# JacobMackay/beifong

Measured on AMD Instinct MI355X. Metric: Mrays/s (closest + any-hit BVH queries), Bus.obj-class radar scene, higher is better.
Workload: dtype f32

## Files before the change

### beifong_amd/csrc/bf_api.cpp

```cpp
#include <hip/hip_runtime.h>

#include <algorithm>
#include <atomic>
#include <cmath>
#include <cstdarg>
#include <cstdio>
#include <cstring>
#include <limits>
#include <memory>
#include <new>
#include <string>
#include <vector>

#include <dlfcn.h>
#if defined(__has_include) && __has_include(<rccl/rccl.h>)
#include <rccl/rccl.h>
#else
extern "C" {
typedef struct ncclComm *ncclComm_t;
typedef enum { ncclSuccess = 0 } ncclResult_t;
typedef enum { ncclFloat = 7 } ncclDataType_t;
typedef enum { ncclSum = 0 } ncclRedOp_t;
ncclResult_t ncclCommInitAll(ncclComm_t *comm, int ndev, const int *devlist);
ncclResult_t ncclCommDestroy(ncclComm_t comm);
// ... 13 lines not shown
#include "bf_wavefront.h"

extern "C" hipError_t bfk_launch_render(const bfd::DScene *sc, const bfd::DLaunch *lp, float *g_hist, bf_path_record *records,
                                        unsigned long long *counters, int stats, unsigned grid, size_t lds_bytes,
                                        hipStream_t stream);
extern "C" float bfk_host_cos(float x);
extern "C" hipError_t bfk_launch_translate(const float4 *tris0, float4 *tris, uint32_t n_tri_rows, const float4 *nodes0,
                                           float4 *nodes, float4 *qnodes, uint32_t n_nodes, const float4 *wnodes0, float4 *wnodes,
                                           uint32_t n_wchildren, const float *d, hipStream_t stream);
extern "C" hipError_t bfk_launch_rigid(const float4 *tris0, float4 *tris, const float4 *nrm0, float4 *nrm, uint32_t n_tris,
                                       const float *xf, const float4 *nodes0, float4 *nodes, float4 *qnodes, uint32_t n_nodes, const uint32_t *lvl4,
                                       const uint32_t *lvl4_off, uint32_t n_lvl4, float4 *ubox4, const float4 *wnodes0, float4 *wnodes, const uint32_t *lvl16,
                                       const uint32_t *lvl16_off, uint32_t n_lvl16, float4 *ubox16, float abs_pad, uint32_t n_versions,
                                       uint64_t vstride, uint32_t xf_stride, hipStream_t stream);
extern "C" hipError_t bfk_launch_elementary(int op, uint64_t n, const float *x, float *y);
extern "C" hipError_t bfk_launch_trace(const bfd::DScene *sc, uint64_t n, const float *rays, int any_hit, float *out_t,
                                       uint32_t *out_prim, uint32_t *out_shape, float *out_uv, uint8_t *out_hit,
                                       float *out_si, hipStream_t stream);
extern "C" hipError_t bfk_launch_query(int op, const bfd::DScene *sc, uint64_t n, const uint32_t *materials, uint32_t emitter,
                                       const float *in, float *out, hipStream_t stream);
extern "C" hipError_t bfk_launch_microfacet(int op, uint32_t type, float alpha_u, float alpha_v, uint32_t sample_visible, uint64_t n,
                                            const float *in, float *out, hipStream_t stream);

extern "C" hipError_t bfk_wf_shade(const bfd::DScene *sc, const bfd::DLaunch *lp, const bfd::WF *wf, uint32_t it, int first,
                                   float *g_hist, bf_path_record *records, unsigned grid, size_t lds_bytes,
                                   hipStream_t stream, int waves);
extern "C" hipError_t bfk_wf_trace(const bfd::DScene *sc, const bfd::WF *wf, uint32_t it, int stats, unsigned grid,
                                   hipStream_t stream, int waves);
extern "C" hipError_t bfk_launch_tail(const bfd::DScene *sc, const bfd::DLaunch *lp, const bfd::WF *wf, uint32_t it,
                                      uint32_t n_slots, float *g_hist, bf_path_record *records, int stats, size_t lds_bytes,
                                      hipStream_t stream, int tail_waves, unsigned spread, unsigned block_cap);
extern "C" hipError_t bfk_roll_set(bfd::DRoll *ring, float4 *offsets, uint32_t idx, const bfd::DRoll *d, const float *offset3, hipStream_t stream);
extern "C" hipError_t bfk_launch_render_fast(const bfd::DScene *sc, const bfd::DLaunch *lp, float *g_hist, bf_path_record *records,
                                             unsigned long long *counters, int stats, unsigned grid, size_t lds_bytes,
                                             hipStream_t stream);
extern "C" hipError_t bfk_wf_shade_fast(const bfd::DScene *sc, const bfd::DLaunch *lp, const bfd::WF *wf, uint32_t it, int first,
                                        float *g_hist, bf_path_record *records, unsigned grid, size_t lds_bytes,
                                        hipStream_t stream, int waves);
extern "C" hipError_t bfk_wf_trace_fast(const bfd::DScene *sc, const bfd::WF *wf, uint32_t it, int stats, unsigned grid,
                                        hipStream_t stream, int waves);
extern "C" hipError_t bfk_launch_tail_fast(const bfd::DScene *sc, const bfd::DLaunch *lp, const bfd::WF *wf, uint32_t it,
                                           uint32_t n_slots, float *g_hist, bf_path_record *records, int stats, size_t lds_bytes,
                                           hipStream_t stream, int tail_waves, unsigned spread, unsigned block_cap);

namespace {
struct Kernels {
    decltype(&bfk_launch_render) render;
    decltype(&bfk_wf_shade) shade;
    decltype(&bfk_wf_trace) trace;
    decltype(&bfk_launch_tail) tail;
};
const Kernels kExact = {bfk_launch_render, bfk_wf_shade, bfk_wf_trace, bfk_launch_tail};
const Kernels kFast = {bfk_launch_render_fast, bfk_wf_shade_fast, bfk_wf_trace_fast, bfk_launch_tail_fast};
const Kernels &kernels_for(uint32_t flags) { return (flags & BF_FLAG_FAST) ? kFast : kExact; }
}

namespace {

thread_local std::string g_err;
// ... 186 lines not shown
        uint32_t window = 1;
        uint32_t iters = 0;
        uint32_t flush_iters = 0;
        uint32_t flush_live = 0;
        bool multi = false;
        uint32_t fb_call_iters = 0;
        bool fb_is_flush = false;
    };
    mutable Roll roll;
    struct TabLayout {
        size_t o_rects = 0, o_shapes = 0, o_emit = 0, o_mat = 0, o_sensor = 0, stride = 0;
    };
    mutable TabLayout tab;
    mutable char *tab_pool = nullptr;
    mutable uint32_t tab_next = 0;
    mutable bool tables_in_pool = false;
    const bfd::DRect *home_rects = nullptr;
    const bfd::DShape *home_shapes = nullptr;
    const bfd::DEmitter *home_emitters = nullptr;
    const bfd::DMaterial *home_materials = nullptr;
    const bfd::DSensor *home_sensor = nullptr;
    mutable bfd::DRoll *roll_ring = nullptr;
    mutable float4 *roll_offsets = nullptr;
    struct WfPlan {
        bool valid = false;
        uint64_t n_paths = 0;
        uint32_t mode = 0, max_depth = 0, n_slots = 0, tail_max = 0;
        uint32_t iters = 0, tail_live = 0;
    };
    mutable WfPlan wf_plan;
    static constexpr int kStageSlots = 8;
    struct Stage {
        void *host = nullptr, *dev = nullptr;
        size_t cap = 0;
        hipEvent_t ev = nullptr;
        bool busy = false;
    };
    mutable Stage stage[kStageSlots];
    mutable int stage_next = 0;
    mutable uint32_t *wf_feedback = nullptr;
    mutable hipEvent_t wf_fb_event = nullptr;
    mutable bool wf_fb_pending = false;
    mutable uint32_t wf_fb_iters = 0;
};

namespace {
// ... 1138 lines not shown
    {
        hipError_t e = hipMalloc((void **) &sc->counters, sizeof(unsigned long long) * bfd::CTR_COUNT);
        if (e == hipSuccess) e = hipMemset(sc->counters, 0, sizeof(unsigned long long) * bfd::CTR_COUNT);
        if (e != hipSuccess) return fail_out(fail(BF_ERR_DEVICE, "bf_scene_clone: counters: %s", hipGetErrorString(e)));
    }
    sc->home_rects = sc->d.rects;
    sc->home_shapes = sc->d.shapes;
    sc->home_emitters = sc->d.emitters;
    sc->home_materials = sc->d.materials;
    sc->home_sensor = sc->d.sensor;
    *out = sc;
    return BF_OK;
}


static bf_status wf_ensure(const bf_scene *scene, uint32_t capacity) {
    bfd::WF &wf = scene->wf;
    if (wf.capacity >= capacity) return BF_OK;
    for (void *p : scene->wf_owned) (void) hipFree(p);
    scene->wf_owned.clear();
    std::memset(&wf, 0, sizeof(wf));
    scene->roll_ring = nullptr;
    scene->roll_offsets = nullptr;
    auto alloc = [&](void **p, size_t bytes) -> hipError_t {
        hipError_t e = hipMalloc(p, bytes);
        if (e == hipSuccess) scene->wf_owned.push_back(*p);
        return e;
    };
    size_t n = capacity, nb = capacity / 64;
#if BF_STATE_AOS
#if BF_STATE_AOS == 2
    HIP_TRY(alloc((void **) &wf.recA, n * 128));
    wf.recB = wf.recA + 4;
#else
    HIP_TRY(alloc((void **) &wf.recA, n * 64));
    HIP_TRY(alloc((void **) &wf.recB, n * 64));
#endif
    HIP_TRY(alloc((void **) &wf.recC, n * 64));
#else
    HIP_TRY(alloc((void **) &wf.ray0_, n * 16));
    HIP_TRY(alloc((void **) &wf.ray1_, n * 16));
    HIP_TRY(alloc((void **) &wf.sa_, n * 16));
    HIP_TRY(alloc((void **) &wf.sb_, n * 16));
    HIP_TRY(alloc((void **) &wf.sd_, n * 16));
    HIP_TRY(alloc((void **) &wf.se_, n * 16));
    HIP_TRY(alloc((void **) &wf.hit_, n * 16));
    HIP_TRY(alloc((void **) &wf.hit_prim_, n * 4));
    HIP_TRY(alloc((void **) &wf.sh0_, n * 16));
    HIP_TRY(alloc((void **) &wf.sh1_, n * 16));
    HIP_TRY(alloc((void **) &wf.sh2_, n * 4));
    HIP_TRY(alloc((void **) &wf.sh3_, n * 4));
    HIP_TRY(alloc((void **) &wf.render_, n * 4));
    HIP_TRY(alloc((void **) &wf.dop_, n * 4));
#endif
    HIP_TRY(alloc((void **) &scene->wf_masks, 8 * nb * sizeof(unsigned long long)));
    HIP_TRY(alloc((void **) &wf.n_live, (bfd::kWfMaxIter + 2) * sizeof(uint32_t)));
    HIP_TRY(alloc((void **) &scene->roll_ring, bfd::kRollRing * sizeof(bfd::DRoll)));
    HIP_TRY(alloc((void **) &scene->roll_offsets, bfd::kRollRing * sizeof(float4)));
    HIP_TRY(alloc((void **) &wf.surv_cursor, 64));
    wf.counters = scene->counters;
    wf.capacity = capacity;
    if (!scene->wf_host) HIP_TRY(hipHostMalloc((void **) &scene->wf_host, 64));
    if (!scene->wf_event) HIP_TRY(hipEventCreateWithFlags(&scene->wf_event, hipEventDisableTiming));
    if (!scene->wf_feedback) HIP_TRY(hipHostMalloc((void **) &scene->wf_feedback, (bfd::kWfMaxIter + 2) * sizeof(uint32_t)));
    if (!scene->wf_fb_event) HIP_TRY(hipEventCreateWithFlags(&scene->wf_fb_event, hipEventDisableTiming));
    scene->wf_plan.valid = false;
    scene->wf_fb_pending = false;
    return BF_OK;
}

static uint32_t wf_tail_threshold(const bf_scene *scene, uint32_t n_slots) {
    if (scene->tun.tail >= 0) return (uint32_t) scene->tun.tail;
    if (n_slots >= bfd::kTailSmallPool) return 1u << 17;
    return std::max<uint32_t>(1u << 17, std::min<uint32_t>(1u << 19, n_slots / 2));
}

namespace {
struct WfCtx {
    const bf_scene *scene;
    const Kernels *k;
    const bfd::DLaunch *lp;
// ... 86 lines not shown
    wf.rf_min = scene->tun.rf_min;
    wf.rf_th = scene->tun.rf_th;
    wf.rf_tm = scene->tun.rf_tm;
    c.lds_shade = ((sizeof(float) * lp.lds_floats + 15) & ~size_t(15)) + (scene->d.tab_cache ? bfd::kTabBytes : 0u);
    c.lds_tail = sizeof(int) * bfd::kStackDepth * bfd::kBlock + c.lds_shade;
    const unsigned batches_per_block = bfd::kBlock / 64;
    const unsigned max_blocks = (unsigned) ((nb + batches_per_block - 1) / batches_per_block);
    c.grid_shade = std::max(1u, std::min((unsigned) scene->n_cus * (unsigned) std::max(2, scene->tun.shade_waves), max_blocks));
    c.grid_trace = std::max(1u, std::min((unsigned) scene->n_cus * (unsigned) scene->tun.trace_waves, max_blocks));
    if (rolling && scene->tun.grid_share > 1u && wf.n_slots < scene->tun.grid_small) {
        const unsigned peers = (unsigned) std::max(1, scene->peers_rolling->load(std::memory_order_relaxed));
        const unsigned share = std::min(peers, (unsigned) scene->tun.grid_share);
        c.grid_shade = std::max(1u, c.grid_shade / share);
        c.grid_trace = std::max(1u, c.grid_trace / share);
    }
    c.tail_max = wf_tail_threshold(scene, rolling ? wf.n_main / 2 : wf.n_slots);
    wf.surv_claims_max = (wf.n_surv / 64u) / std::max(1u, c.grid_shade * batches_per_block);
    if (rolling && scene->tun.debug_surv_batches) {
        const char *e = getenv("BF_DEBUG_SURV_CLAIMS");
        wf.surv_claims_max = e ? (uint32_t) strtoul(e, nullptr, 10) : 1u << 20;
    }
    return BF_OK;
}
static bf_status wf_iteration(const WfCtx &c, uint32_t it, int first) {
    const bf_scene *scene = c.scene;
    const bfd::WF &wf = scene->wf;
    const int nxt = (it & 1) ^ 1;
    HIP_TRY(hipMemsetAsync(wf.m_alive[nxt], 0, c.mask_bytes, c.stream));
    if (first != 1) {
        HIP_TRY(wf_tic(c, 1));
        HIP_TRY(c.k->shade(&scene->d, c.lp, &wf, it, first == 2 ? 3 : 0, c.hist, c.rec, c.grid_shade, c.lds_shade, c.stream,
                           scene->tun.shade_waves));
        HIP_TRY(wf_toc(c));
    }
    if (first != 0) {
        HIP_TRY(wf_tic(c, 1));
        HIP_TRY(c.k->shade(&scene->d, c.lp, &wf, it, first, c.hist, c.rec, c.grid_shade, c.lds_shade, c.stream, scene->tun.shade_waves));
        HIP_TRY(wf_toc(c));
    }
    return BF_OK;
}
static bf_status wf_trace_launch(const WfCtx &c, uint32_t it) {
    HIP_TRY(wf_tic(c, 0));
    HIP_TRY(c.k->trace(&c.scene->d, &c.scene->wf, it, c.count_nodes ? 1 : 0, c.grid_trace, c.stream, c.scene->tun.trace_waves));
    HIP_TRY(wf_toc(c));
    return BF_OK;
}
static bf_status wf_tail_launch(const WfCtx &c, uint32_t it, uint32_t est_live, bool alone = false) {
    const bf_scene *scene = c.scene;
    uint32_t share = 1;
    if (!alone && scene->tun.tail_share > 1) {
        share = scene->tun.tail_share >= 4 ? 4u : 2u;
        est_live = (uint32_t) std::min<uint64_t>((uint64_t) est_live * share, 1u << 30);
    }
    if (alone) {
        const uint32_t resident = (uint32_t) scene->n_cus * 4u * 3u;
        while (share < 4u && (uint64_t) est_live * (share * 2u) / 64u <= resident) share *= 2u;
        est_live = (uint32_t) std::min<uint64_t>((uint64_t) est_live * share, 1u << 30);
    }
    scene->wf.tail_share = share;
// ... 1416 lines not shown
```

### beifong_amd/csrc/bf_device_core.h

```cpp
#pragma once
#include "bf_device.h"
#include "bf_device_math.h"

BF_NS_BEGIN

struct Hit {
    float t, u, v;
    uint32_t prim;
    int32_t slot;
};

BF_DEV bool tri_intersect(V3 p0, V3 p1, V3 p2, V3 o, V3 d, float mint, float maxt, float &t, float &u, float &v) {
    V3 e1 = p1 - p0, e2 = p2 - p0;
    V3 pvec = cross(d, e2);
    float inv_det = rcp(dot(e1, pvec));
    V3 tvec = o - p0;
    u = dot(tvec, pvec) * inv_det;
    bool active = u >= 0.f && u <= 1.f;
    V3 qvec = cross(tvec, e1);
    v = dot(d, qvec) * inv_det;
    active = active && v >= 0.f && u + v <= 1.f;
    t = dot(e2, qvec) * inv_det;
    return active && t >= mint && t <= maxt;
}
// ... 696 lines not shown
        }
        if (FULL) {
            geom->n = n;
            geom->dp_du = dp_du;
            geom->dp_dv = dp_dv;
        }
        if (tag & 1u) {
            si.sh.n = normalize(mk(na.x, na.y, na.z) * b0 + mk(nb.x, nb.y, nb.z) * b1 + mk(nc.x, nc.y, nc.z) * b2);
        } else {
            si.sh.n = n;
        }
    }
    float dd = dot(si.sh.n, dp_du);
    si.sh.s = normalize(mk(fnmadd(si.sh.n.x, dd, dp_du.x), fnmadd(si.sh.n.y, dd, dp_du.y), fnmadd(si.sh.n.z, dd, dp_du.z)));
    si.sh.t = cross(si.sh.n, si.sh.s);
    si.wi = to_local(si.sh, -d);
}

struct Microfacet {
    uint32_t type;
    float au, av;
    bool sample_visible;
};
BF_DEV void load_tables_lds(DScene &sc, uint32_t byte_off, uint32_t tid) {
    extern __shared__ __align__(16) unsigned char s_dyn[];
    sc.tab_on = 0u;
    if (!sc.tab_cache) return;
    float *dst = reinterpret_cast<float *>(s_dyn + byte_off);
    const float *gm = reinterpret_cast<const float *>(sc.materials), *gr = reinterpret_cast<const float *>(sc.rects);
    for (uint32_t i = tid; i < sc.n_materials * 12u; i += kBlock) dst[i] = gm[i];
    for (uint32_t i = tid; i < sc.n_rects * kRectDwords; i += kBlock) dst[kTabMaxMaterials * 12u + i] = gr[i];
    sc.lds_mat = byte_off;
    sc.lds_rect = byte_off + kTabMaxMaterials * 48u;
    sc.tab_on = 1u;
}
BF_DEV bf_material load_material(const DScene &sc, uint32_t index) {
    bf_f4 a, b, c;
    if (sc.tab_on) {
        extern __shared__ __align__(16) unsigned char s_dyn[];
        const lds_f4_ptr mp = (lds_f4_ptr) (s_dyn + sc.lds_mat) + 3u * index;
        a = mp[0], b = mp[1], c = mp[2];
    } else {
        const c_f4_ptr mp = (c_f4_ptr) (uintptr_t) (sc.materials + index);
        a = mp[0], b = mp[1], c = mp[2];
    }
    bf_material m;
    m.type = __float_as_uint(a.x);
    m.twosided = __float_as_uint(a.y);
    m.reflectance = a.z;
    m.alpha_u = a.w;
    m.alpha_v = b.x;
    m.distribution = __float_as_uint(b.y);
    m.sample_visible = __float_as_uint(b.z);
    m.eta = b.w;
    m.k = c.x;
    m.has_specular_reflectance = __float_as_uint(c.y);
    m.back_material = __float_as_uint(c.z);
// ... 338 lines not shown
```

### beifong_amd/csrc/bf_kernels.hip

```cpp
#include <algorithm>
#include <cstring>

#include "bf_path_logic.h"

BF_NS_BEGIN

#ifndef BF_TAIL_WAVES
#define BF_TAIL_WAVES 3
#endif
#ifdef BF_TAIL_PROF
__device__ unsigned long long g_tail_prof[8192 * 24];
#define BF_PROF_STAMP(var) const unsigned long long var = __builtin_amdgcn_s_memtime()
#else
#define BF_PROF_STAMP(var)
#endif
template <bool STATS, bool RESUME, bool SPILL, int TW = BF_TAIL_WAVES, int VX = 0>
__global__ __launch_bounds__(kBlock, RESUME ? TW : 3) void bf_render_kernel(DScene sc_arg, DLaunch lp, float *__restrict__ g_hist,
                                                           bf_path_record *__restrict__ records,
                                                           unsigned long long *__restrict__ counters, WF wf, uint32_t wf_it) {
    constexpr int kRX = 2 | VX;
    extern __shared__ __align__(16) unsigned char s_raw[];
    int *s_stack = reinterpret_cast<int *>(s_raw);
    float *s_hist = reinterpret_cast<float *>(s_raw + sizeof(int) * kStackDepth * kBlock);
    const int tid = threadIdx.x;
// ... 559 lines not shown
    if (MODE >= 1) row = (g * 2654435761u) & (n - 1u);
    if (MODE == 2) row *= 8u;
    const float4 v = table[row];
    if (v.x == 12345.678f) out[g & 1023u] = v;
}
BF_NS_END
extern "C" hipError_t bfk_gather_probe(int mode, const float4 *table, uint32_t n_rows, float4 *out, hipStream_t stream) {
    const uint32_t n = mode == 2 ? n_rows / 8u : n_rows;
    const dim3 grid((n + 255u) / 256u), block(256);
    if (mode == 0) hipLaunchKernelGGL(bfd::bf_gather_probe<0>, grid, block, 0, stream, table, n_rows, out);
    else if (mode == 1) hipLaunchKernelGGL(bfd::bf_gather_probe<1>, grid, block, 0, stream, table, n_rows, out);
    else hipLaunchKernelGGL(bfd::bf_gather_probe<2>, grid, block, 0, stream, table, n_rows, out);
    return hipGetLastError();
}

BF_NS_BEGIN
__global__ void bf_roll_set_kernel(DRoll *ring, float4 *offsets, uint32_t idx, DRoll d, float4 off) {
    if (threadIdx.x == 0 && blockIdx.x == 0) {
        ring[idx] = d;
        offsets[idx] = off;
    }
}
BF_NS_END
extern "C" hipError_t bfk_roll_set(bfd::DRoll *ring, float4 *offsets, uint32_t idx, const bfd::DRoll *d, const float *offset3, hipStream_t stream) {
    const float4 off = offset3 ? make_float4(offset3[0], offset3[1], offset3[2], 0.f) : make_float4(0.f, 0.f, 0.f, 0.f);
    hipLaunchKernelGGL(bfd::bf_roll_set_kernel, dim3(1), dim3(64), 0, stream, ring, offsets, idx, *d, off);
    return hipGetLastError();
}

BF_NS_BEGIN
BF_DEV void quantise_node4_dev(float4 lx, float4 ly, float4 lz, float4 hx, float4 hy, float4 hz, float4 refs, float4 *__restrict__ q) {
    const float cl[3][4] = {{lx.x, lx.y, lx.z, lx.w}, {ly.x, ly.y, ly.z, ly.w}, {lz.x, lz.y, lz.z, lz.w}};
    const float chh[3][4] = {{hx.x, hx.y, hx.z, hx.w}, {hy.x, hy.y, hy.z, hy.w}, {hz.x, hz.y, hz.z, hz.w}};
    const int child[4] = {__float_as_int(refs.x), __float_as_int(refs.y), __float_as_int(refs.z), __float_as_int(refs.w)};
    float nlo[3], scale[3];
    uint32_t exps = 0, qlo[3] = {0, 0, 0}, qhi[3] = {0, 0, 0};
    for (int a = 0; a < 3; ++a) {
        float lo = BF_INF, hi = -BF_INF;
        for (int k = 0; k < 4; ++k)
            if (child[k] != kNoNode) {
                lo = __builtin_fminf(lo, cl[a][k]);
                hi = __builtin_fmaxf(hi, chh[a][k]);
            }
        nlo[a] = lo;
        int e = 0;
        (void) __builtin_frexpf((hi - lo) * (1.f / 255.f), &e);
// ... 438 lines not shown
```

### beifong_amd/csrc/bf_wavefront.h

```cpp
#pragma once
#include <hip/hip_runtime.h>

#include "bf_ns.h"
#include <stdint.h>

BF_NS_BEGIN

constexpr uint32_t kWfMaxIter = 4096;
constexpr uint32_t kShadeChain = 8;
constexpr uint32_t kTraceRefill = 32;
constexpr uint32_t kTraceStragglers = 12;
constexpr uint32_t kTraceBlocksPerCU = 8;
constexpr uint32_t kTailSmallPool = 1u << 22;
constexpr uint32_t kTailRowJobs = 12;

#ifndef BF_STATE_AOS
#define BF_STATE_AOS 1
#endif
#define BF_HD __host__ __device__ __forceinline__

struct WF {
#if BF_STATE_AOS
    static constexpr size_t kAB = BF_STATE_AOS == 2 ? 8 : 4;
    float4 *recA, *recB, *recC;
    BF_HD float4 &ray0(uint32_t i) const { return recA[kAB * (size_t) i + 0]; }
    BF_HD float4 &ray1(uint32_t i) const { return recA[kAB * (size_t) i + 1]; }
    BF_HD float4 &hit(uint32_t i) const { return recA[kAB * (size_t) i + 2]; }
// ... 35 lines not shown
    uint32_t geom_stride;
    unsigned long long *m_alive[2];
    unsigned long long *m_trace[2];
    unsigned long long *m_shadow[2];
    unsigned long long *m_hit[2];
    uint32_t hit_split;
    uint32_t chain_min;
    uint32_t rf_min, rf_th, rf_tm;
    uint32_t *n_live;
    unsigned long long *counters;
    uint32_t trace_refill, trace_stragglers;
    uint32_t iq;
    uint32_t shade_chain;
    uint32_t row_jobs;
    uint32_t n_slots;
    uint32_t capacity;
    uint32_t n_main, n_surv;
    uint32_t *surv_cursor;
    uint32_t wake_b0, wake_nb;
    uint32_t tail_share;
    uint32_t surv_claims_max;
};

BF_NS_END
```

### beifong_amd/csrc/bf_wavefront.hip

```cpp
#include "bf_path_logic.h"

BF_NS_BEGIN

BF_DEV void publish_masks(unsigned long long *m_out, bool aligned, bool merge, uint32_t batch0, uint32_t slot, bool valid_lane, bool bit) {
    if (aligned) {
        unsigned long long w = __ballot(bit);
        if ((threadIdx.x & 63) == 0 && w) {
            if (merge)
                atomicOr(&m_out[batch0], w);
            else
                m_out[batch0] = w;
        }
    } else if (valid_lane && bit) {
        atomicOr(&m_out[slot >> 6], 1ull << (slot & 63u));
    }
}

constexpr uint32_t kPublishGroups = 4;
BF_DEV void publish_grouped(volatile unsigned char *tr, int lane, bool settle, uint32_t slot, uint32_t bits, unsigned long long *m_alive,
                            unsigned long long *m_trace, unsigned long long *m_shadow) {
    unsigned long long todo = __ballot(settle && bits != 0u);
    for (uint32_t n = 0; todo != 0ull && n < kPublishGroups; ++n) {
        const int j = __ffsll(todo) - 1;
        const uint32_t b = (uint32_t) __shfl((int) (slot >> 6), j);
// ... 79 lines not shown
            sv.free = 0ull;
        } else {
            const uint32_t p = nth_set_bit(sv.free, take - 1u);
            sv.free &= ~((2ull << p) - 1ull);
        }
        served += take;
    }
    if (evict && rank >= served) evict = false;
}

#ifdef BF_SHADE_PROF
#define SLT(k)                                                            \
    do {                                                                  \
        const unsigned long long slt_now = __builtin_amdgcn_s_memtime();  \
        t_sec[k] += slt_now - slt_last;                                   \
        slt_last = slt_now;                                               \
    } while (0)
#else
#define SLT(k)
#endif
#ifndef BF_SHADE_REFILL
#define BF_SHADE_REFILL 0
#endif
template <int FIRST, int W, int RX>
__global__ __launch_bounds__(kBlock, W) void wf_shade(DScene sc_arg, DLaunch lp, WF wf, uint32_t it, float *__restrict__ g_hist,
                                                      bf_path_record *__restrict__ records) {
    extern __shared__ __align__(16) unsigned char s_raw[];
    float *s_hist = reinterpret_cast<float *>(s_raw);
    const int tid = threadIdx.x, lane = tid & 63;
    DScene sc = sc_arg;
    if (RX & kMulti) sc.tab_cache = 0u;
    load_tables_lds(sc, (4u * lp.lds_floats + 15u) & ~15u, (uint32_t) tid);
    constexpr bool WALK = FIRST == 0 || FIRST == 3;
    constexpr bool EVICT = FIRST == 3;
    const bool lds_hist = lp.lds_hist != 0;
    if (lp.lds_floats || sc.tab_on) {
        for (uint32_t i = tid; i < lp.lds_floats; i += kBlock) s_hist[i] = 0.f;
        __syncthreads();
    }
    const int cur = it & 1, nxt = cur ^ 1;
    const bool receive = mode_receive<RX>(lp);
    if (FIRST == 2 && blockIdx.x == 0 && tid == 0) {
        wf.surv_cursor[0] += wf.surv_cursor[1];
        wf.surv_cursor[1] = 0u;
    }
    const uint32_t n_batches = WALK ? wf.n_slots >> 6 : (FIRST == 2 ? wf.wake_nb : wf.n_main >> 6);
    unsigned long long *m_alive = wf.m_alive[nxt], *m_trace = wf.m_trace[nxt], *m_shadow = wf.m_shadow[nxt], *m_hit = wf.m_hit[nxt];
    SurvAlloc sv = {0ull, 0u, 0u, EVICT ? wf.surv_cursor[0] : 0u};

    FilmAcc acc = {0.f, 0.f, 0.f, 0.f, 0.f, 0u, 0u};
    uint32_t c_closest = 0, c_shadow = 0, c_bounces = 0, c_live = 0, c_traced = 0, c_loads = 0, c_shq = 0;
#ifdef BF_SHADE_PROF
    const bool lpf = BF_SHADE_PROF >= 2;
    ShadeProf spf = {0, 0, 0, 0};
    unsigned long long t_sec[8] = {0, 0, 0, 0, 0, 0, 0, 0};
// ... 16 lines not shown
        cursor_init(cur_alive, wf.m_alive[cur], wave_id, n_waves, n_batches, lane);
    else if (FIRST == 2)
        cursor_init(cur_alive, m_alive, wave_id, n_waves, wf.wake_nb, lane, 1u, nullptr, 0u, wf.wake_b0, wf.n_main >> 6, 1u);
    else
        cursor_init(cur_alive, nullptr, wave_id, n_waves, wf.n_main >> 6, lane);
    const unsigned long long lt_mask = (1ull << lane) - 1ull;
    bool has = false, have_hit = false, need_film = false, need_gen = false, touched = false;
    uint32_t slot = 0, rounds = 0, guard = 0;
    PathState s;
    s.render = 0u;
    s.flags = 0u;
    s.path_i = 0ull;
    ShadowReq sh;
    sh.want = false;
    Hit hit;
    hit.t = BF_INF;
    hit.u = hit.v = 0.f;
    hit.prim = 0;
    hit.slot = 0;
    bool done = false;
    uint32_t out_bits = 0u;
    const uint32_t rf_min = wf.rf_min, rf_th = wf.rf_th, rf_tm = wf.rf_tm;
    while (true) {
        const bool pend_any = has && !done;
        const unsigned long long xm = __ballot(!pend_any);
        if ((uint32_t) __popcll(xm) >= rf_min || xm == ~0ull) {
            if (__any(done)) {
                const bool keep = done && out_bits != 0u;
                const bool tracing = (out_bits & 2u) != 0u, shadowing = (out_bits & 4u) != 0u;
                bool evict = false;
                uint32_t dst = slot;
                SLP(20, keep);
                if (EVICT) {
                    const uint32_t main_b = wf.n_main >> 6, b = slot >> 6;
                    const uint32_t rel = b >= wf.wake_b0 ? b - wf.wake_b0 : b + main_b - wf.wake_b0;
                    evict = keep && slot < wf.n_main && rel < wf.wake_nb && s.path_i + wf.n_main < lp.n_paths;
                    const unsigned long long em = __ballot(evict);
                    if (em) surv_take(wf, cur, sv, em, evict, dst, lane);
                    if (evict) wf.sd(slot) = make_uint4(0u, 0u, (uint32_t) s.path_i, (uint32_t) (s.path_i >> 32));
                }
                if (keep) {
                    if (!(s.flags & kFlagTermPending)) {
                        wf.hit(dst) = make_float4(hit.t, hit.u, hit.v, __int_as_float(hit.slot));
                        wf.hit_prim(dst) = hit.prim;
                    }
                    store_state(wf, dst, receive, s);
// ... 138 lines not shown
                bool found;
                tracing = presolve_ray(scp, false, s.ro, s.rd, s.rmint, s.rmaxt, hit, found, shf);
            }
        }
        SLT(4);
        const bool resolved = go && cont && !tracing && !shadowing;
        const bool chain = resolved && rounds + 1u < wf.shade_chain;
        if (go) ++rounds;
        if (chain) {
            if (s.flags & kFlagTermPending)
                need_film = true;
            else
                have_hit = true;
        }
        if (go && !chain && (cont || fin)) {
            done = true;
            out_bits = cont ? (1u | (tracing ? 2u : 0u) | (shadowing ? 4u : 0u)) : 0u;
        }
    }
#else
    for (uint32_t pass = 0; pass < n_pass; ++pass) {
    if (WALK) cursor_init(cur_alive, wf.m_alive[cur], wave_id, n_waves, n_batches, lane, 1u, n_pass == 2u ? wf.m_hit[cur] : nullptr, pass ? 1u : 2u);
    while (true) {
        uint32_t slot = 0, got;
        bool aligned;
        if (!WALK) {
            if (first_b >= n_batches) break;
            uint32_t fb = first_b;
            if (FIRST == 2) {
                fb += wf.wake_b0;
                if (fb >= wf.n_main >> 6) fb -= wf.n_main >> 6;
            }
            slot = fb * 64u + lane;
            got = 64;
            aligned = true;
            first_b += n_waves;
        } else {
            cursor_skip_empty(cur_alive, lane);
            if (cursor_empty(cur_alive)) break;
            const uint32_t batch_before = cur_alive.b;
            const bool whole = __popcll(cur_alive.m) == 64;
            got = cursor_take(cur_alive, 64u, true, (uint32_t) lane, slot, lane);
            if (got == 0) break;
            aligned = whole && got == 64 && slot == batch_before * 64u + (uint32_t) lane;
            aligned = __all(aligned);
        }
// ... 27 lines not shown
                ++c_loads;
                SLP(1, (s.flags & kFlagTermPending) != 0);
                if (s.flags & kFlagTermPending) {
                    film_put<RX>(sc, lp, s, s_hist, g_hist, lds_hist, acc, records);
                    need_gen = true;
                } else {
                    float4 hq = wf.hit(slot);
                    hit.t = hq.x;
                    hit.u = hq.y;
                    hit.v = hq.z;
                    hit.slot = __float_as_int(hq.w);
                    have_hit = true;
                }
            }
        }
#ifdef BF_SHADE_PROF
        asm volatile("s_waitcnt vmcnt(0)" ::: "memory");
#endif
        SLT(1);
        bool settled = !has;
        bool touched = FIRST != 2;
        bool tracing = false, shadowing = false;
        for (uint32_t round = 0;; ++round) {
            SLP(2 + min(round, 2u), !settled && have_hit);
            if (!settled && have_hit) {
                have_hit = false;
#ifdef BF_SHADE_PROF
                cont = shade_vertex<RX>(sc, lp, s, hit, sh, c_bounces, &spf, lpf);
#else
                cont = shade_vertex<RX>(sc, lp, s, hit, sh, c_bounces);
#endif
                SLT(7);
                SLP(5, !cont);
                if (!cont) {
                    film_put<RX>(sc, lp, s, s_hist, g_hist, lds_hist, acc, records);
                    need_gen = true;
                } else if (!(s.flags & kFlagTermPending)) {
                    ++c_closest;
                }
                if (sh.want) ++c_shadow;
            }
            SLT(2);
            SLP(6, !settled && need_gen);
            if (!settled && need_gen) {
                need_gen = false;
                cont = false;
// ... 80 lines not shown
        }
        cont = has && cont;
        tracing = cont && tracing;
        shadowing = cont && shadowing;
        publish_masks(m_alive, aligned, FIRST == 2, batch0, slot, has, cont && !evict);
        publish_masks(m_trace, aligned, FIRST == 2, batch0, slot, has, tracing && !evict);
        publish_masks(m_shadow, aligned, FIRST == 2, batch0, slot, has, shadowing && !evict);
        const bool hit_known = cont && !tracing && !(s.flags & kFlagTermPending) && hit.t != BF_INF;
        if (wf.hit_split) publish_masks(m_hit, aligned, FIRST == 2, batch0, slot, has, hit_known && !evict);
        if (evict) {
            const unsigned long long bit = 1ull << (dst & 63u);
            atomicOr(&m_alive[dst >> 6], bit);
            if (tracing) atomicOr(&m_trace[dst >> 6], bit);
            if (shadowing) atomicOr(&m_shadow[dst >> 6], bit);
            if (wf.hit_split && hit_known) atomicOr(&m_hit[dst >> 6], bit);
        }
        c_traced += (tracing ? 1u : 0u) + (shadowing ? 1u : 0u);
        c_shq += shadowing ? 1u : 0u;
        SLT(6);
    }
    }
#endif

    film_flush<RX>(lp, acc, s_hist, g_hist, lds_hist, tid);
#ifdef BF_SHADE_PROF
#pragma unroll
    for (int off = 32; off > 0; off >>= 1) {
        spf.si = max(spf.si, (unsigned long long) __shfl_down((long long) spf.si, off));
        spf.head = max(spf.head, (unsigned long long) __shfl_down((long long) spf.head, off));
        spf.nee = max(spf.nee, (unsigned long long) __shfl_down((long long) spf.nee, off));
        spf.bsdf = max(spf.bsdf, (unsigned long long) __shfl_down((long long) spf.bsdf, off));
    }
    if (lane == 0) {
        for (int k = 0; k < 8; ++k) atomicAdd(&g_lane_prof[24 + k], t_sec[k]);
        atomicAdd(&g_lane_prof[kShadeProfSections + 24], spf.si);
        atomicAdd(&g_lane_prof[kShadeProfSections + 25], spf.head);
        atomicAdd(&g_lane_prof[kShadeProfSections + 26], spf.nee);
        atomicAdd(&g_lane_prof[kShadeProfSections + 27], spf.bsdf);
    }
#endif
    unsigned long long v_closest = c_closest, v_shadow = c_shadow, v_invalid = acc.invalid, v_bounces = c_bounces;
    uint32_t v_live = c_live, v_film = acc.n_put;
    unsigned long long v_traced = c_traced;
    uint32_t v_loads = c_loads, v_shq = c_shq;
#pragma unroll
    for (int off = 32; off > 0; off >>= 1) {
// ... 7 lines not shown
        v_live += __shfl_down(v_live, off);
        v_film += __shfl_down(v_film, off);
    }
    __shared__ uint32_t s_live[kBlock / 64];
    if (lane == 0) s_live[tid >> 6] = v_live;
    __syncthreads();
    if (tid == 0) {
        uint32_t t = 0;
        for (int k = 0; k < kBlock / 64; ++k) t += s_live[k];
        if (t) atomicAdd(&wf.n_live[it], t);
    }
    if (lane == 0 && lp.count) {
        if (v_film) atomicAdd(&wf.counters[CTR_FILM], (unsigned long long) v_film);
        if (v_closest) atomicAdd(&wf.counters[CTR_CLOSEST], v_closest);
        if (v_shadow) atomicAdd(&wf.counters[CTR_SHADOW], v_shadow);
        if (v_invalid) atomicAdd(&wf.counters[CTR_INVALID], v_invalid);
        if (v_bounces) atomicAdd(&wf.counters[CTR_BOUNCES], v_bounces);
        if (v_traced) atomicAdd(&wf.counters[CTR_TRACED], v_traced);
        if (v_loads) atomicAdd(&wf.counters[CTR_SHADE_LOADS], (unsigned long long) v_loads);
        if (v_live) atomicAdd(&wf.counters[CTR_SHADE_STORES], (unsigned long long) v_live);
        if (v_shq) atomicAdd(&wf.counters[CTR_SHADE_SHADOW], (unsigned long long) v_shq);
        if (v_closest + v_shadow) atomicAdd(&wf.counters[CTR_SHADE_RAYS], v_closest + v_shadow);
    }
}

constexpr int kLdsStack = 16;
#ifndef BF_TRACE_IFIF
#define BF_TRACE_IFIF 0
#endif
constexpr uint32_t kTraceGuard = 1u << 24;

template <bool STATS, int W, bool SHIFT, bool QUANT, bool GEOM = false>
__global__ __launch_bounds__(kBlock, W) void wf_trace(DScene sc, WF wf, uint32_t it) {
    __shared__ int s_stack[kLdsStack * kBlock];
    __shared__ float4 s_top[kTopNodes * (QUANT ? kTopStrideQ : kTopStride)];
    int *stack = s_stack + threadIdx.x;
    const int lane = threadIdx.x & 63;
    const int nxt = (it & 1) ^ 1;
    uint32_t c_nodes = 0, c_tris = 0, c_top = 0;
    const int n_top = GEOM ? 0 : (int) min(sc.n_nodes, kTopNodes);
    if (QUANT && !GEOM)
        load_top_qnodes(sc.qnodes, (uint32_t) n_top, s_top, threadIdx.x, kBlock);
    else if (!GEOM)
        load_top_nodes(sc.nodes, (uint32_t) n_top, s_top, threadIdx.x, kBlock);
    __syncthreads();
    const uint32_t n_waves = gridDim.x * (kBlock / 64), wave_id = blockIdx.x * (kBlock / 64) + (threadIdx.x >> 6);
    LaneStack<kLdsStack, true> st = make_stack<kLdsStack, true>(sc, stack);
// ... 201 lines not shown
        if (lane == 0) {
            atomicAdd(&wf.counters[CTR_NODES], v_nodes);
            atomicAdd(&wf.counters[CTR_TRIS], v_tris);
            atomicAdd(&wf.counters[CTR_NODES_LDS], v_top);
        }
    }
}

BF_NS_END

#ifdef BF_SHADE_PROF
extern "C" int bfdbg_shade_lane_profile(unsigned long long *out, int clear) {
    if (hipDeviceSynchronize() != hipSuccess) return -1;
    if (out && hipMemcpyFromSymbol(out, HIP_SYMBOL(bfd::g_lane_prof), sizeof(unsigned long long) * 2 * bfd::kShadeProfSections) != hipSuccess) return -1;
    if (clear) {
        void *p = nullptr;
        if (hipGetSymbolAddress(&p, HIP_SYMBOL(bfd::g_lane_prof)) != hipSuccess) return -1;
        if (hipMemset(p, 0, sizeof(unsigned long long) * 2 * bfd::kShadeProfSections) != hipSuccess) return -1;
    }
    return 2 * bfd::kShadeProfSections;
}
#endif

extern "C" hipError_t BF_LAUNCHER(bfk_wf_shade)(const bfd::DScene *sc, const bfd::DLaunch *lp, const bfd::WF *wf, uint32_t it, int first,
                                   float *g_hist, bf_path_record *records, unsigned grid, size_t lds_bytes,
                                   hipStream_t stream, int waves) {
    const bool rx = lp->mode == BF_MODE_RECEIVE_RAW;
#define BF_SHADE_LAUNCH_RX(F, W, RX_)                                                                                              \
    hipLaunchKernelGGL((bfd::wf_shade<F, W, RX_>), dim3(grid), dim3(bfd::kBlock), lds_bytes, stream, *sc, *lp, *wf, it, g_hist, records)
#define BF_SHADE_LAUNCH(F, W)            \
    if (rx) BF_SHADE_LAUNCH_RX(F, W, 1); \
    else BF_SHADE_LAUNCH_RX(F, W, 0)
#define BF_SHADE_LAUNCH_WIDE(F)                          \
    if (rx) BF_SHADE_LAUNCH_RX(F, 3, 1 | bfd::kWide);    \
    else BF_SHADE_LAUNCH_RX(F, 3, 0 | bfd::kWide)
#define BF_SHADE_LAUNCH_LEAN(F)                          \
    if (rx) BF_SHADE_LAUNCH_RX(F, 3, 1 | bfd::kLean);    \
    else BF_SHADE_LAUNCH_RX(F, 3, 0 | bfd::kLean)
#define BF_SHADE_LAUNCH_MULTI(F)                         \
    if (rx) BF_SHADE_LAUNCH_RX(F, 3, 1 | bfd::kMulti);   \
    else BF_SHADE_LAUNCH_RX(F, 3, 0 | bfd::kMulti)
#define BF_SHADE_LAUNCH_GEOM(F, V)                           \
    if (rx) BF_SHADE_LAUNCH_RX(F, 3, 1 | bfd::kGeom | (V));  \
    else BF_SHADE_LAUNCH_RX(F, 3, 0 | bfd::kGeom | (V))
#define BF_SHADE_LAUNCH_GEOM_V(F)                                          \
    if (lp->lean && !lp->wide) { BF_SHADE_LAUNCH_GEOM(F, bfd::kLean); }    \
    else if (lp->wide) { BF_SHADE_LAUNCH_GEOM(F, bfd::kWide); }            \
    else { BF_SHADE_LAUNCH_GEOM(F, 0); }
    if (lp->geom_stride) {
        if (first >= 2) return hipErrorInvalidValue;
        if (first) { BF_SHADE_LAUNCH_GEOM_V(1); }
        else { BF_SHADE_LAUNCH_GEOM_V(0); }
    } else if (lp->multi) {
        if (first == 3) { BF_SHADE_LAUNCH_MULTI(3); }
        else if (first == 2) { BF_SHADE_LAUNCH_MULTI(2); }
        else if (first) { BF_SHADE_LAUNCH_MULTI(1); }
        else { BF_SHADE_LAUNCH_MULTI(0); }
    } else if (lp->lean && !lp->wide && (first || waves == 3)) {
        if (first == 3) { BF_SHADE_LAUNCH_LEAN(3); }
        else if (first == 2) { BF_SHADE_LAUNCH_LEAN(2); }
        else if (first) { BF_SHADE_LAUNCH_LEAN(1); }
        else { BF_SHADE_LAUNCH_LEAN(0); }
    } else if (lp->wide) {
        if (first == 3) { BF_SHADE_LAUNCH_WIDE(3); }
        else if (first == 2) { BF_SHADE_LAUNCH_WIDE(2); }
        else if (first) { BF_SHADE_LAUNCH_WIDE(1); }
        else { BF_SHADE_LAUNCH_WIDE(0); }
    } else if (first == 3) {
        BF_SHADE_LAUNCH(3, 3);
    } else if (first == 2) {
        BF_SHADE_LAUNCH(2, 3);
    } else if (first) {
        BF_SHADE_LAUNCH(1, 3);
    } else {
        switch (waves) {
            case 2: BF_SHADE_LAUNCH(0, 2); break;
// ... 67 lines not shown
```

Baseline: 1670.

## Pass shade kernel arguments through a device buffer instead of by value

Replaces the large by-value DScene/DLaunch/WF kernel arguments of wf_shade with a pointer to a device-resident ShadeArgs struct. The struct is filled on the host, precomputes LDS table offsets, and is uploaded by a tiny kernel only when its contents change. Inside the kernel the struct is re-read through a constant address-space pointer at each loop scope, so scalar registers are not kept live across the shading loops. This aims to cut register pressure and per-launch argument traffic, at the cost of repeated scalar loads and one extra small launch whenever the arguments change.

```diff
diff --git a/beifong_amd/csrc/bf_api.cpp b/beifong_amd/csrc/bf_api.cpp
--- a/beifong_amd/csrc/bf_api.cpp
+++ b/beifong_amd/csrc/bf_api.cpp
@@ -59,7 +59,7 @@
 extern "C" hipError_t bfk_launch_microfacet(int op, uint32_t type, float alpha_u, float alpha_v, uint32_t sample_visible, uint64_t n,
                                             const float *in, float *out, hipStream_t stream);
 
-extern "C" hipError_t bfk_wf_shade(const bfd::DScene *sc, const bfd::DLaunch *lp, const bfd::WF *wf, uint32_t it, int first,
+extern "C" hipError_t bfk_wf_shade(const bfd::ShadeArgs *args, const bfd::DLaunch *lp, uint32_t it, int first,
                                    float *g_hist, bf_path_record *records, unsigned grid, size_t lds_bytes,
                                    hipStream_t stream, int waves);
 extern "C" hipError_t bfk_wf_trace(const bfd::DScene *sc, const bfd::WF *wf, uint32_t it, int stats, unsigned grid,
@@ -68,10 +68,11 @@
                                       uint32_t n_slots, float *g_hist, bf_path_record *records, int stats, size_t lds_bytes,
                                       hipStream_t stream, int tail_waves, unsigned spread, unsigned block_cap);
 extern "C" hipError_t bfk_roll_set(bfd::DRoll *ring, float4 *offsets, uint32_t idx, const bfd::DRoll *d, const float *offset3, hipStream_t stream);
+extern "C" hipError_t bfk_shade_args_set(bfd::ShadeArgs *dst, const bfd::ShadeArgs *a, hipStream_t stream);
 extern "C" hipError_t bfk_launch_render_fast(const bfd::DScene *sc, const bfd::DLaunch *lp, float *g_hist, bf_path_record *records,
                                              unsigned long long *counters, int stats, unsigned grid, size_t lds_bytes,
                                              hipStream_t stream);
-extern "C" hipError_t bfk_wf_shade_fast(const bfd::DScene *sc, const bfd::DLaunch *lp, const bfd::WF *wf, uint32_t it, int first,
+extern "C" hipError_t bfk_wf_shade_fast(const bfd::ShadeArgs *args, const bfd::DLaunch *lp, uint32_t it, int first,
                                         float *g_hist, bf_path_record *records, unsigned grid, size_t lds_bytes,
                                         hipStream_t stream, int waves);
 extern "C" hipError_t bfk_wf_trace_fast(const bfd::DScene *sc, const bfd::WF *wf, uint32_t it, int stats, unsigned grid,
@@ -304,6 +305,9 @@
     const bfd::DSensor *home_sensor = nullptr;
     mutable bfd::DRoll *roll_ring = nullptr;
     mutable float4 *roll_offsets = nullptr;
+    mutable bfd::ShadeArgs *shade_args = nullptr;
+    mutable bfd::ShadeArgs shade_args_last;
+    mutable bool shade_args_valid = false;
     struct WfPlan {
         bool valid = false;
         uint64_t n_paths = 0;
@@ -1488,6 +1492,8 @@
     std::memset(&wf, 0, sizeof(wf));
     scene->roll_ring = nullptr;
     scene->roll_offsets = nullptr;
+    scene->shade_args = nullptr;
+    scene->shade_args_valid = false;
     auto alloc = [&](void **p, size_t bytes) -> hipError_t {
         hipError_t e = hipMalloc(p, bytes);
         if (e == hipSuccess) scene->wf_owned.push_back(*p);
@@ -1523,6 +1529,7 @@
     HIP_TRY(alloc((void **) &wf.n_live, (bfd::kWfMaxIter + 2) * sizeof(uint32_t)));
     HIP_TRY(alloc((void **) &scene->roll_ring, bfd::kRollRing * sizeof(bfd::DRoll)));
     HIP_TRY(alloc((void **) &scene->roll_offsets, bfd::kRollRing * sizeof(float4)));
+    HIP_TRY(alloc((void **) &scene->shade_args, sizeof(bfd::ShadeArgs)));
     HIP_TRY(alloc((void **) &wf.surv_cursor, 64));
     wf.counters = scene->counters;
     wf.capacity = capacity;
@@ -1655,20 +1662,36 @@
     }
     return BF_OK;
 }
+static hipError_t shade_args_sync(const WfCtx &c) {
+    const bf_scene *scene = c.scene;
+    bfd::ShadeArgs a;
+    std::memset(&a, 0, sizeof(a));
+    std::memcpy(&a.sc, &scene->d, sizeof(a.sc));
+    std::memcpy(&a.lp, c.lp, sizeof(a.lp));
+    std::memcpy(&a.wf, &scene->wf, sizeof(a.wf));
+    bfd::shade_tables(a);
+    if (scene->shade_args_valid && std::memcmp(&a, &scene->shade_args_last, sizeof(a)) == 0) return hipSuccess;
+    const hipError_t e = bfk_shade_args_set(scene->shade_args, &a, c.stream);
+    if (e != hipSuccess) return e;
+    std::memcpy(&scene->shade_args_last, &a, sizeof(a));
+    scene->shade_args_valid = true;
+    return hipSuccess;
+}
 static bf_status wf_iteration(const WfCtx &c, uint32_t it, int first) {
     const bf_scene *scene = c.scene;
     const bfd::WF &wf = scene->wf;
     const int nxt = (it & 1) ^ 1;
     HIP_TRY(hipMemsetAsync(wf.m_alive[nxt], 0, c.mask_bytes, c.stream));
+    HIP_TRY(shade_args_sync(c));
     if (first != 1) {
         HIP_TRY(wf_tic(c, 1));
-        HIP_TRY(c.k->shade(&scene->d, c.lp, &wf, it, first == 2 ? 3 : 0, c.hist, c.rec, c.grid_shade, c.lds_shade, c.stream,
+        HIP_TRY(c.k->shade(scene->shade_args, c.lp, it, first == 2 ? 3 : 0, c.hist, c.rec, c.grid_shade, c.lds_shade, c.stream,
                            scene->tun.shade_waves));
         HIP_TRY(wf_toc(c));
     }
     if (first != 0) {
         HIP_TRY(wf_tic(c, 1));
-        HIP_TRY(c.k->shade(&scene->d, c.lp, &wf, it, first, c.hist, c.rec, c.grid_shade, c.lds_shade, c.stream, scene->tun.shade_waves));
+        HIP_TRY(c.k->shade(scene->shade_args, c.lp, it, first, c.hist, c.rec, c.grid_shade, c.lds_shade, c.stream, scene->tun.shade_waves));
         HIP_TRY(wf_toc(c));
     }
     return BF_OK;
diff --git a/beifong_amd/csrc/bf_device_core.h b/beifong_amd/csrc/bf_device_core.h
--- a/beifong_amd/csrc/bf_device_core.h
+++ b/beifong_amd/csrc/bf_device_core.h
@@ -742,17 +742,19 @@
     float au, av;
     bool sample_visible;
 };
-BF_DEV void load_tables_lds(DScene &sc, uint32_t byte_off, uint32_t tid) {
+BF_DEV void copy_tables_lds(const DScene &sc, uint32_t tid) {
     extern __shared__ __align__(16) unsigned char s_dyn[];
-    sc.tab_on = 0u;
-    if (!sc.tab_cache) return;
-    float *dst = reinterpret_cast<float *>(s_dyn + byte_off);
+    if (!sc.tab_on) return;
+    float *dst = reinterpret_cast<float *>(s_dyn + sc.lds_mat);
     const float *gm = reinterpret_cast<const float *>(sc.materials), *gr = reinterpret_cast<const float *>(sc.rects);
     for (uint32_t i = tid; i < sc.n_materials * 12u; i += kBlock) dst[i] = gm[i];
     for (uint32_t i = tid; i < sc.n_rects * kRectDwords; i += kBlock) dst[kTabMaxMaterials * 12u + i] = gr[i];
+}
+BF_DEV void load_tables_lds(DScene &sc, uint32_t byte_off, uint32_t tid) {
+    sc.tab_on = sc.tab_cache ? 1u : 0u;
     sc.lds_mat = byte_off;
     sc.lds_rect = byte_off + kTabMaxMaterials * 48u;
-    sc.tab_on = 1u;
+    copy_tables_lds(sc, tid);
 }
 BF_DEV bf_material load_material(const DScene &sc, uint32_t index) {
     bf_f4 a, b, c;
diff --git a/beifong_amd/csrc/bf_kernels.hip b/beifong_amd/csrc/bf_kernels.hip
--- a/beifong_amd/csrc/bf_kernels.hip
+++ b/beifong_amd/csrc/bf_kernels.hip
@@ -605,6 +605,15 @@
     }
 }
 BF_NS_END
+BF_NS_BEGIN
+__global__ void bf_shade_args_kernel(ShadeArgs *dst, ShadeArgs a) {
+    if (threadIdx.x == 0 && blockIdx.x == 0) *dst = a;
+}
+BF_NS_END
+extern "C" hipError_t bfk_shade_args_set(bfd::ShadeArgs *dst, const bfd::ShadeArgs *a, hipStream_t stream) {
+    hipLaunchKernelGGL(bfd::bf_shade_args_kernel, dim3(1), dim3(64), 0, stream, dst, *a);
+    return hipGetLastError();
+}
 extern "C" hipError_t bfk_roll_set(bfd::DRoll *ring, float4 *offsets, uint32_t idx, const bfd::DRoll *d, const float *offset3, hipStream_t stream) {
     const float4 off = offset3 ? make_float4(offset3[0], offset3[1], offset3[2], 0.f) : make_float4(0.f, 0.f, 0.f, 0.f);
     hipLaunchKernelGGL(bfd::bf_roll_set_kernel, dim3(1), dim3(64), 0, stream, ring, offsets, idx, *d, off);
diff --git a/beifong_amd/csrc/bf_wavefront.h b/beifong_amd/csrc/bf_wavefront.h
--- a/beifong_amd/csrc/bf_wavefront.h
+++ b/beifong_amd/csrc/bf_wavefront.h
@@ -3,6 +3,8 @@
 
 #include "bf_ns.h"
 #include <stdint.h>
+
+#include "bf_device.h"
 
 BF_NS_BEGIN
 
@@ -84,4 +86,16 @@
     uint32_t surv_claims_max;
 };
 
+struct ShadeArgs {
+    DScene sc;
+    DLaunch lp;
+    WF wf;
+};
+BF_HD bool shade_multi(const DLaunch &lp) { return lp.geom_stride == 0u && lp.multi != 0u; }
+inline void shade_tables(ShadeArgs &a) {
+    a.sc.tab_on = a.sc.tab_cache && !shade_multi(a.lp) ? 1u : 0u;
+    a.sc.lds_mat = a.sc.tab_on ? (4u * a.lp.lds_floats + 15u) & ~15u : 0u;
+    a.sc.lds_rect = a.sc.tab_on ? a.sc.lds_mat + kTabMaxMaterials * 48u : 0u;
+}
+
 BF_NS_END
diff --git a/beifong_amd/csrc/bf_wavefront.hip b/beifong_amd/csrc/bf_wavefront.hip
--- a/beifong_amd/csrc/bf_wavefront.hip
+++ b/beifong_amd/csrc/bf_wavefront.hip
@@ -125,15 +125,28 @@
 #ifndef BF_SHADE_REFILL
 #define BF_SHADE_REFILL 0
 #endif
+typedef const BF_CAS ShadeArgs CShadeArgs;
+BF_DEV const ShadeArgs &shade_args(CShadeArgs *p) {
+    asm volatile("" : "+s"(p));
+    return *(const ShadeArgs *) p;
+}
+#define BF_SHADE_ARGS()                           \
+    const ShadeArgs &args_ = shade_args(ka);      \
+    const DScene &sc = args_.sc;                  \
+    const DLaunch &lp = args_.lp;                 \
+    const WF &wf = args_.wf;                      \
+    (void) sc;                                    \
+    (void) lp;                                    \
+    (void) wf
 template <int FIRST, int W, int RX>
-__global__ __launch_bounds__(kBlock, W) void wf_shade(DScene sc_arg, DLaunch lp, WF wf, uint32_t it, float *__restrict__ g_hist,
+__global__ __launch_bounds__(kBlock, W) void wf_shade(const ShadeArgs *args, uint32_t it, float *__restrict__ g_hist,
                                                       bf_path_record *__restrict__ records) {
     extern __shared__ __align__(16) unsigned char s_raw[];
     float *s_hist = reinterpret_cast<float *>(s_raw);
     const int tid = threadIdx.x, lane = tid & 63;
-    DScene sc = sc_arg;
-    if (RX & kMulti) sc.tab_cache = 0u;
-    load_tables_lds(sc, (4u * lp.lds_floats + 15u) & ~15u, (uint32_t) tid);
+    CShadeArgs *const ka = as_const(args);
+    BF_SHADE_ARGS();
+    copy_tables_lds(sc, (uint32_t) tid);
     constexpr bool WALK = FIRST == 0 || FIRST == 3;
     constexpr bool EVICT = FIRST == 3;
     const bool lds_hist = lp.lds_hist != 0;
@@ -196,6 +209,7 @@
     uint32_t out_bits = 0u;
     const uint32_t rf_min = wf.rf_min, rf_th = wf.rf_th, rf_tm = wf.rf_tm;
     while (true) {
+        BF_SHADE_ARGS();
         const bool pend_any = has && !done;
         const unsigned long long xm = __ballot(!pend_any);
         if ((uint32_t) __popcll(xm) >= rf_min || xm == ~0ull) {
@@ -380,6 +394,7 @@
     for (uint32_t pass = 0; pass < n_pass; ++pass) {
     if (WALK) cursor_init(cur_alive, wf.m_alive[cur], wave_id, n_waves, n_batches, lane, 1u, n_pass == 2u ? wf.m_hit[cur] : nullptr, pass ? 1u : 2u);
     while (true) {
+        BF_SHADE_ARGS();
         uint32_t slot = 0, got;
         bool aligned;
         if (!WALK) {
@@ -453,6 +468,7 @@
         bool touched = FIRST != 2;
         bool tracing = false, shadowing = false;
         for (uint32_t round = 0;; ++round) {
+            BF_SHADE_ARGS();
             SLP(2 + min(round, 2u), !settled && have_hit);
             if (!settled && have_hit) {
                 have_hit = false;
@@ -579,6 +595,8 @@
     }
 #endif
 
+    {
+    BF_SHADE_ARGS();
     film_flush<RX>(lp, acc, s_hist, g_hist, lds_hist, tid);
 #ifdef BF_SHADE_PROF
 #pragma unroll
@@ -632,7 +650,9 @@
         if (v_shq) atomicAdd(&wf.counters[CTR_SHADE_SHADOW], (unsigned long long) v_shq);
         if (v_closest + v_shadow) atomicAdd(&wf.counters[CTR_SHADE_RAYS], v_closest + v_shadow);
     }
+    }
 }
+#undef BF_SHADE_ARGS
 
 constexpr int kLdsStack = 16;
 #ifndef BF_TRACE_IFIF
@@ -880,12 +900,12 @@
 }
 #endif
 
-extern "C" hipError_t BF_LAUNCHER(bfk_wf_shade)(const bfd::DScene *sc, const bfd::DLaunch *lp, const bfd::WF *wf, uint32_t it, int first,
+extern "C" hipError_t BF_LAUNCHER(bfk_wf_shade)(const bfd::ShadeArgs *args, const bfd::DLaunch *lp, uint32_t it, int first,
                                    float *g_hist, bf_path_record *records, unsigned grid, size_t lds_bytes,
                                    hipStream_t stream, int waves) {
     const bool rx = lp->mode == BF_MODE_RECEIVE_RAW;
 #define BF_SHADE_LAUNCH_RX(F, W, RX_)                                                                                              \
-    hipLaunchKernelGGL((bfd::wf_shade<F, W, RX_>), dim3(grid), dim3(bfd::kBlock), lds_bytes, stream, *sc, *lp, *wf, it, g_hist, records)
+    hipLaunchKernelGGL((bfd::wf_shade<F, W, RX_>), dim3(grid), dim3(bfd::kBlock), lds_bytes, stream, args, it, g_hist, records)
 #define BF_SHADE_LAUNCH(F, W)            \
     if (rx) BF_SHADE_LAUNCH_RX(F, W, 1); \
     else BF_SHADE_LAUNCH_RX(F, W, 0)
@@ -909,7 +929,7 @@
         if (first >= 2) return hipErrorInvalidValue;
         if (first) { BF_SHADE_LAUNCH_GEOM_V(1); }
         else { BF_SHADE_LAUNCH_GEOM_V(0); }
-    } else if (lp->multi) {
+    } else if (bfd::shade_multi(*lp)) {
         if (first == 3) { BF_SHADE_LAUNCH_MULTI(3); }
         else if (first == 2) { BF_SHADE_LAUNCH_MULTI(2); }
         else if (first) { BF_SHADE_LAUNCH_MULTI(1); }
```

Measured after the change: 1681, median of 6. About the same (+0.7%).
